# rain-neuromorphics/torchmx

Hardware: NVIDIA B200
Metric: to_mx/to_dtype GB/s (algorithmic bytes: quantize + dequantize->bf16, 16384x16384 bf16, all elem dtypes, block 32) (higher is better)
Workload: dtype u8 codes / f32 scaling arithmetic

## Files before the change

include/mxq.h:

```cpp
#ifndef MXQ_H_
#define MXQ_H_

#include <stdint.h>

#if defined(__GNUC__)
#define MXQ_API __attribute__((visibility("default")))
#else
#define MXQ_API
#endif

#ifdef __cplusplus
extern "C" {
#endif

typedef enum {
    MXQ_ELEM_E4M3 = 0,
    MXQ_ELEM_E3M2 = 1,
    MXQ_ELEM_E2M3 = 2,
    MXQ_ELEM_E2M1 = 3,
    MXQ_ELEM_INT8 = 4,
    MXQ_ELEM_E5M2 = 5
} mxq_elem_t;

typedef enum {
// ... 123 lines not shown
typedef struct {
    const void *x; int64_t n0, n1, rows, cols, s0, s1, row_stride;
    int elem ; unsigned flags ;
    void *codes; uint8_t *scales;
} mxq_transposed_quantize_args_t;
MXQ_API int mxq_quantize_transposed(const mxq_transposed_quantize_args_t *args, int device, void *stream);

#define MXQ_OK 0
#define MXQ_ERR_INVALID 1
#define MXQ_ERR_UNSUPPORTED_SHAPE 2
#define MXQ_ERR_CUDA 3

MXQ_API const char *mxq_last_error(void);
MXQ_API int mxq_version(void);
MXQ_API int mxq_arch(void);

#ifdef __cplusplus
}
#endif
#endif
```

torchmx_b200/_C.py:

```python
from __future__ import annotations

import ctypes
import os
import threading

_HERE = os.path.dirname(os.path.abspath(__file__))
LIB_PATH = os.path.join(_HERE, "lib", "libmxq.so")

OK, ERR_INVALID, ERR_UNSUPPORTED_SHAPE, ERR_CUDA = 0, 1, 2, 3
HP_BF16, HP_F32 = 0, 1
FLAG_HW_EXACT = 1
FLAG_OPERAND_LAYOUT = 2
GEMM_B_STATIC, GEMM_WIDE_TILES, GEMM_NO_PDL, GEMM_NO_MXF4 = 1, 2, 4, 8
ABI_VERSION = 3
MAX_DIMS = 6

EXPORTS = ("mxq_quantize", "mxq_dequantize", "mxq_dequantize_strided", "mxq_gemm", "mxq_gemm_dequant", "mxq_gemm_bf16", "mxq_transcode_to_e4m3", "mxq_pack_operand", "mxq_unpack_operand",
           "mxq_softmax_quantize", "mxq_flash_attention", "mxq_silu_mul_quantize", "mxq_rmsnorm", "mxq_rope", "mxq_quantize_heads", "mxq_quantize_transposed", "mxq_last_error", "mxq_version", "mxq_arch")


class GemmArgs(ctypes.Structure):
    _fields_ = [
        ("a_codes", ctypes.c_void_p), ("sfa", ctypes.c_void_p), ("lda", ctypes.c_int64), ("ld_sfa", ctypes.c_int64),
        ("a_batch_stride", ctypes.c_int64), ("sfa_batch_stride", ctypes.c_int64),
        ("b_codes", ctypes.c_void_p), ("sfb", ctypes.c_void_p), ("ldb", ctypes.c_int64), ("ld_sfb", ctypes.c_int64),
        ("b_batch_stride", ctypes.c_int64), ("sfb_batch_stride", ctypes.c_int64),
        ("bias", ctypes.c_void_p),
        ("d", ctypes.c_void_p), ("ldd", ctypes.c_int64), ("d_batch_stride", ctypes.c_int64),
        ("batch", ctypes.c_int64), ("M", ctypes.c_int64), ("N", ctypes.c_int64), ("K", ctypes.c_int64),
        ("a_format", ctypes.c_int), ("b_format", ctypes.c_int),
        ("d_multicast", ctypes.c_void_p),
        ("x_bf16", ctypes.c_void_p), ("ldx", ctypes.c_int64), ("x_quant_flags", ctypes.c_int),
        ("flags", ctypes.c_uint), ("split_k", ctypes.c_int),
# ... 90 lines not shown
    if _lib is not None:
        return _lib
    with _lock:
        if _lib is not None:
            return _lib
        if not os.path.exists(LIB_PATH):
            raise RuntimeError(
                f"torchmx_b200: {LIB_PATH} is missing. Build it with `python -m torchmx_b200.build` "
                "(needs nvcc; sm_100a). There is no CPU / PyTorch fallback for the MX kernels.")
        L = ctypes.CDLL(LIB_PATH)
        i64, i32, vp, u32 = ctypes.c_int64, ctypes.c_int, ctypes.c_void_p, ctypes.c_uint
        L.mxq_last_error.restype = ctypes.c_char_p
        L.mxq_last_error.argtypes = []
        L.mxq_version.restype = i32
        L.mxq_arch.restype = i32
        L.mxq_quantize.restype = i32
        L.mxq_quantize.argtypes = [vp, i32, i64, i32, i32, u32, vp, vp, i32, vp]
        L.mxq_dequantize.restype = i32
        L.mxq_dequantize.argtypes = [vp, vp, i64, i32, i32, i32, vp, i32, vp]
        L.mxq_dequantize_strided.restype = i32
        L.mxq_dequantize_strided.argtypes = [vp, vp, i32, ctypes.POINTER(i64), ctypes.POINTER(i64), ctypes.POINTER(i64),
                                             i32, i32, i32, i32, vp, i32, vp]
        L.mxq_gemm.restype = i32
        L.mxq_gemm.argtypes = [ctypes.POINTER(GemmArgs), i32, vp]
        L.mxq_gemm_dequant.restype = i32
        L.mxq_gemm_dequant.argtypes = [ctypes.POINTER(GemmDequantArgs), i32, vp]
        L.mxq_gemm_bf16.restype = i32
        L.mxq_gemm_bf16.argtypes = [vp, i64, i64, vp, i64, i64, vp, vp, i64, i64, i64, i64, i64, i64, i32, vp]
        L.mxq_transcode_to_e4m3.restype = i32
        L.mxq_transcode_to_e4m3.argtypes = [vp, i32, i64, vp, i32, vp]
# ... 34 lines not shown
```

torchmx_b200/csrc/mxq_api.cu:

```cuda
#include <cstdarg>
#include <cstdio>
#include <cstdlib>
#include <cstring>

#include "mxq_common.cuh"

namespace mxq {
cudaError_t launch_quantize(const void*, int, int64_t, int, int, unsigned, void*, uint8_t*, int, int, int, cudaStream_t);
cudaError_t launch_dequantize(const void*, const uint8_t*, int64_t, int, int, int, void*, int, int, int, cudaStream_t);
cudaError_t launch_dequantize_strided(const void*, const uint8_t*, int, const int64_t*, const int64_t*, const int64_t*, int, int, int, int,
                                      void*, cudaStream_t);
cudaError_t launch_transcode(const void*, int, int64_t, void*, int, cudaStream_t);
cudaError_t launch_pack_operand(const void*, int, int64_t, void*, int, cudaStream_t);
cudaError_t launch_unpack_operand(const void*, int, int64_t, void*, int, cudaStream_t);
int launch_gemm(const mxq_gemm_args_t*, int, int, cudaStream_t, char*, size_t);
namespace gemm { int launch_gemm_dequant(const mxq_gemm_dequant_args_t*, int, cudaStream_t, char*, size_t); }
namespace gemm { int launch_gemm_bf16(const void*, int64_t, int64_t, const void*, int64_t, int64_t, const void*, void*, int64_t, int64_t, int64_t, int64_t, int64_t, int64_t, int,
                                       cudaStream_t, char*, size_t); }
namespace gemm { int launch_flash_attention(const mxq_attention_args_t*, int, cudaStream_t, char*, size_t); }
cudaError_t launch_silu_mul_quantize(const void*, const void*, int64_t, int64_t, int64_t, int64_t, int, unsigned, void*, uint8_t*, int, cudaStream_t);
int launch_softmax_quantize(const mxq_softmax_args_t*, cudaStream_t, char*, size_t);
int launch_rmsnorm(const mxq_rmsnorm_args_t*, cudaStream_t, char*, size_t);
int launch_rope(const mxq_rope_args_t*, int, cudaStream_t, char*, size_t);
int launch_heads_quantize(const void*, int64_t, int64_t, int64_t, int64_t, int, unsigned, void*, uint8_t*, cudaStream_t, char*, size_t);
// ... 29 lines not shown
        if (prev >= 0 && cur != prev) cudaSetDevice(prev);
    }
};

int sm_count_of(int device) {
    static int cache[64];
    if (device >= 0 && device < 64 && cache[device]) return cache[device];
    int n = 0;
    if (cudaDeviceGetAttribute(&n, cudaDevAttrMultiProcessorCount, device) != cudaSuccess || n <= 0) n = 148;
    if (device >= 0 && device < 64) cache[device] = n;
    return n;
}

bool valid_elem(int e) { return e >= MXQ_ELEM_E4M3 && e <= MXQ_ELEM_E5M2; }

int env_int(const char* name) {
    const char* s = getenv(name);
    return s ? atoi(s) : 0;
}
int quant_ept_override() { static int v = env_int("MXQ_QUANT_EPT"); return (v == 8 || v == 16 || v == 32) ? v : 0; }
int deq_cb_override() { static int v = env_int("MXQ_DEQ_CB"); return (v == 16 || v == 32) ? v : 0; }
int waves_override() { static int v = env_int("MXQ_WAVES"); return v > 0 ? v : 0; }

}

extern "C" {

const char* mxq_last_error(void) { return g_err; }
int mxq_version(void) { return 3; }
int mxq_arch(void) { return 1000; }

int mxq_quantize(const void* src, int src_dtype, int64_t n_blocks, int block_size, int elem, unsigned flags, void* codes, uint8_t* scales,
                 int device, void* stream) {
    if (!valid_elem(elem)) return fail(MXQ_ERR_INVALID, "mxq_quantize: unknown element type %d", elem);
    if (src_dtype != MXQ_HP_BF16 && src_dtype != MXQ_HP_F32) return fail(MXQ_ERR_INVALID, "mxq_quantize: unsupported source dtype %d", src_dtype);
    if (n_blocks < 0 || block_size < 1) return fail(MXQ_ERR_INVALID, "mxq_quantize: bad n_blocks=%lld block_size=%d", (long long)n_blocks, block_size);
    if (n_blocks == 0) return MXQ_OK;
    if (!src || !codes || !scales) return fail(MXQ_ERR_INVALID, "mxq_quantize: null pointer");
    if (elem == MXQ_ELEM_E2M1 && ((n_blocks * block_size) & 1))
        return fail(MXQ_ERR_INVALID, "mxq_quantize: float4_e2m1 needs an even element count (got %lld)", (long long)(n_blocks * block_size));
    DeviceScope scope(device);
    if (scope.err != cudaSuccess) return fail_cuda(scope.err, "mxq_quantize: selecting device");
    const cudaError_t e = mxq::launch_quantize(src, src_dtype, n_blocks, block_size, elem, flags, codes, scales, sm_count_of(scope.cur),
                                               quant_ept_override(), waves_override(), (cudaStream_t)stream);
    if (e == cudaErrorNotSupported && (flags & MXQ_FLAG_OPERAND_LAYOUT))
        return fail(MXQ_ERR_UNSUPPORTED_SHAPE, "mxq_quantize: MXQ_FLAG_OPERAND_LAYOUT needs a 4 / 6-bit element type, block 32, bf16 source and 32-byte aligned pointers");
    return e == cudaSuccess ? MXQ_OK : fail_cuda(e, "mxq_quantize: launch");
}

int mxq_dequantize(const void* codes, const uint8_t* scales, int64_t n_blocks, int block_size, int elem, int dst_dtype, void* dst, int device,
                   void* stream) {
    if (!valid_elem(elem)) return fail(MXQ_ERR_INVALID, "mxq_dequantize: unknown element type %d", elem);
    if (dst_dtype != MXQ_HP_BF16 && dst_dtype != MXQ_HP_F32) return fail(MXQ_ERR_INVALID, "mxq_dequantize: unsupported target dtype %d", dst_dtype);
    if (n_blocks < 0 || block_size < 1) return fail(MXQ_ERR_INVALID, "mxq_dequantize: bad n_blocks=%lld block_size=%d", (long long)n_blocks, block_size);
    if (n_blocks == 0) return MXQ_OK;
    if (!codes || !scales || !dst) return fail(MXQ_ERR_INVALID, "mxq_dequantize: null pointer");
    if (elem == MXQ_ELEM_E2M1 && ((n_blocks * block_size) & 1)) return fail(MXQ_ERR_INVALID, "mxq_dequantize: float4_e2m1 needs an even element count");
    DeviceScope scope(device);
    if (scope.err != cudaSuccess) return fail_cuda(scope.err, "mxq_dequantize: selecting device");
    const cudaError_t e = mxq::launch_dequantize(codes, scales, n_blocks, block_size, elem, dst_dtype, dst, sm_count_of(scope.cur), deq_cb_override(), waves_override(),
                                                 (cudaStream_t)stream);
    return e == cudaSuccess ? MXQ_OK : fail_cuda(e, "mxq_dequantize: launch");
}

int mxq_dequantize_strided(const void* codes, const uint8_t* scales, int ndim, const int64_t* sizes, const int64_t* code_strides,
                           const int64_t* scale_strides, int block_dim, int block_size, int elem, int dst_dtype, void* dst, int device,
                           void* stream) {
    if (!valid_elem(elem)) return fail(MXQ_ERR_INVALID, "mxq_dequantize_strided: unknown element type %d", elem);
    if (dst_dtype != MXQ_HP_BF16 && dst_dtype != MXQ_HP_F32) return fail(MXQ_ERR_INVALID, "mxq_dequantize_strided: unsupported target dtype %d", dst_dtype);
    if (ndim < 1 || ndim > MXQ_MAX_DIMS) return fail(MXQ_ERR_INVALID, "mxq_dequantize_strided: ndim %d outside 1..%d", ndim, MXQ_MAX_DIMS);
    if (block_dim < 0 || block_dim >= ndim || block_size < 1) return fail(MXQ_ERR_INVALID, "mxq_dequantize_strided: bad block_dim=%d block_size=%d", block_dim, block_size);
    if (!sizes || !code_strides || !scale_strides) return fail(MXQ_ERR_INVALID, "mxq_dequantize_strided: null shape pointer");
    int64_t total = 1;
    for (int d = 0; d < ndim; ++d) {
        if (sizes[d] < 0) return fail(MXQ_ERR_INVALID, "mxq_dequantize_strided: negative size");
        total *= sizes[d];
// ... 189 lines not shown
```

torchmx_b200/csrc/mxq_common.cuh:

```cuda
#pragma once
#include <cstdlib>
#include <cstdint>
#include <cuda_runtime.h>

#include "../../include/mxq.h"

namespace mxq {

template <int ELEM> struct Fmt;
template <> struct Fmt<MXQ_ELEM_E4M3> { static constexpr int ebits = 4, mbits = 3, bias = 7, max_pow2 = 8; };
template <> struct Fmt<MXQ_ELEM_E3M2> { static constexpr int ebits = 3, mbits = 2, bias = 3, max_pow2 = 4; };
template <> struct Fmt<MXQ_ELEM_E2M3> { static constexpr int ebits = 2, mbits = 3, bias = 1, max_pow2 = 2; };
template <> struct Fmt<MXQ_ELEM_E2M1> { static constexpr int ebits = 2, mbits = 1, bias = 1, max_pow2 = 2; };
template <> struct Fmt<MXQ_ELEM_INT8> { static constexpr int ebits = 0, mbits = 7, bias = 0, max_pow2 = 6; };
template <> struct Fmt<MXQ_ELEM_E5M2> { static constexpr int ebits = 5, mbits = 2, bias = 15, max_pow2 = 15; };

struct alignas(32) u32x8 { uint32_t v[8]; };

__device__ __forceinline__ u32x8 ldg256_stream(const void* p) {
    u32x8 r;
    asm volatile("ld.global.nc.L1::no_allocate.v8.b32 {%0,%1,%2,%3,%4,%5,%6,%7}, [%8];"
                 : "=r"(r.v[0]), "=r"(r.v[1]), "=r"(r.v[2]), "=r"(r.v[3]), "=r"(r.v[4]), "=r"(r.v[5]), "=r"(r.v[6]), "=r"(r.v[7])
                 : "l"(p));
    return r;
// ... 7 lines not shown
    uint2 r;
    asm volatile("ld.global.nc.L1::no_allocate.v2.b32 {%0,%1}, [%2];" : "=r"(r.x), "=r"(r.y) : "l"(p));
    return r;
}
__device__ __forceinline__ void stg256_stream(void* p, const u32x8& r) {
    asm volatile("st.global.L1::no_allocate.v8.b32 [%0], {%1,%2,%3,%4,%5,%6,%7,%8};" ::"l"(p), "r"(r.v[0]), "r"(r.v[1]), "r"(r.v[2]),
                 "r"(r.v[3]), "r"(r.v[4]), "r"(r.v[5]), "r"(r.v[6]), "r"(r.v[7])
                 : "memory");
}
__device__ __forceinline__ void stg128_stream(void* p, uint4 r) {
    asm volatile("st.global.L1::no_allocate.v4.b32 [%0], {%1,%2,%3,%4};" ::"l"(p), "r"(r.x), "r"(r.y), "r"(r.z), "r"(r.w) : "memory");
}
__device__ __forceinline__ void stg64_stream(void* p, uint2 r) {
    asm volatile("st.global.L1::no_allocate.v2.b32 [%0], {%1,%2};" ::"l"(p), "r"(r.x), "r"(r.y) : "memory");
}

template <int ELEM>
__device__ __forceinline__ int shared_exp_from_maxE(int maxE) {
    int s = maxE - Fmt<ELEM>::max_pow2;
    s = max(s, 0);
    s = min(s, 254);
    return maxE == 255 ? 255 : s;
}
__device__ __forceinline__ float inv_scale_f32(int s) {
    return __uint_as_float(s <= 253 ? (uint32_t)(254 - s) << 23 : 0x00400000u);
}
__device__ __forceinline__ float scale_f32(int s) {
    return __uint_as_float(s == 0 ? 0x00400000u : (s == 255 ? 0x7FC00000u : (uint32_t)s << 23));
}

// ... 105 lines not shown
```

torchmx_b200/csrc/mxq_dequantize.cu:

```cuda
#include <type_traits>

#include "mxq_common.cuh"

namespace mxq {

constexpr int kDequantThreads = 256;

template <int ELEM>
__device__ __forceinline__ void decode4(uint32_t word, float sc, float (&f)[4]) {
    if constexpr (ELEM == MXQ_ELEM_INT8) {
#pragma unroll
        for (int j = 0; j < 4; ++j) f[j] = (float)(int)(int8_t)(word >> (8 * j)) * sc;
    } else {
        const uint32_t h0 = decode_pair_f16x2<ELEM>(word & 0xFFFF), h1 = decode_pair_f16x2<ELEM>(word >> 16);
        f[0] = f16lo_to_f32(h0) * sc; f[1] = f16hi_to_f32(h0) * sc;
        f[2] = f16lo_to_f32(h1) * sc; f[3] = f16hi_to_f32(h1) * sc;
    }
}

__device__ __forceinline__ void decode8_e2m1(uint32_t word, float sc, float (&f)[8]) {
#pragma unroll
    for (int j = 0; j < 4; ++j) {
        const uint32_t h = decode_e2m1_byte_f16x2((word >> (8 * j)) & 0xFF);
        f[2 * j] = f16hi_to_f32(h) * sc;
        f[2 * j + 1] = f16lo_to_f32(h) * sc;
    }
}

template <int N, bool F32>
__device__ __forceinline__ void store_run(void* dst, int64_t first_elem, const float (&f)[N]) {
    if constexpr (F32) {
        uint8_t* p = reinterpret_cast<uint8_t*>(dst) + first_elem * 4;
#pragma unroll
        for (int j = 0; j < N / 8; ++j) {
            u32x8 o;
#pragma unroll
            for (int k = 0; k < 8; ++k) o.v[k] = __float_as_uint(f[8 * j + k]);
            stg256_stream(p + 32 * j, o);
        }
    } else {
        uint8_t* p = reinterpret_cast<uint8_t*>(dst) + first_elem * 2;
#pragma unroll
        for (int j = 0; j < N / 16; ++j) {
            u32x8 o;
#pragma unroll
            for (int k = 0; k < 8; ++k) o.v[k] = pack_bf16x2(f[16 * j + 2 * k], f[16 * j + 2 * k + 1]);
            stg256_stream(p + 32 * j, o);
        }
    }
}

template <int ELEM, bool F32, int CB>
__global__ void __launch_bounds__(kDequantThreads) dequantize_b32_kernel(const uint8_t* __restrict__ codes, const uint8_t* __restrict__ scales,
                                                                         void* __restrict__ dst, int64_t n_code_bytes) {
    constexpr int PER = (ELEM == MXQ_ELEM_E2M1) ? 2 : 1;
    constexpr int NH = CB / 16;
    const int64_t n_chunks = n_code_bytes / CB;
    const int64_t stride = (int64_t)gridDim.x * kDequantThreads;
    for (int64_t c = (int64_t)blockIdx.x * kDequantThreads + threadIdx.x; c < n_chunks; c += stride) {
        uint32_t w[CB / 4];
        if constexpr (CB == 32) {
            const u32x8 v = ldg256_stream(codes + c * 32);
#pragma unroll
            for (int k = 0; k < 8; ++k) w[k] = v.v[k];
        } else {
            const uint4 v = ldg128_stream(codes + c * 16);
            w[0] = v.x; w[1] = v.y; w[2] = v.z; w[3] = v.w;
        }
        int s[NH];
#pragma unroll
        for (int h = 0; h < NH; ++h) s[h] = __ldg(scales + ((c * CB + 16 * h) * PER) / 32);
#pragma unroll
        for (int h = 0; h < NH; ++h) {
            const float sc = scale_f32(s[h]);
            const int64_t e0 = (c * CB + 16 * h) * PER;
            if constexpr (ELEM == MXQ_ELEM_E2M1) {
                float f[32];
#pragma unroll
                for (int i = 0; i < 4; ++i) {
                    float t[8];
                    decode8_e2m1(w[4 * h + i], sc, t);
#pragma unroll
                    for (int k = 0; k < 8; ++k) f[8 * i + k] = t[k];
                }
                store_run<32, F32>(dst, e0, f);
            } else {
                float f[16];
#pragma unroll
                for (int i = 0; i < 4; ++i) {
                    float t[4];
                    decode4<ELEM>(w[4 * h + i], sc, t);
#pragma unroll
                    for (int k = 0; k < 4; ++k) f[4 * i + k] = t[k];
                }
                store_run<16, F32>(dst, e0, f);
            }
        }
    }
}

struct StridedArgs {
    int ndim, block_dim, block_size;
    int64_t sizes[MXQ_MAX_DIMS], code_strides[MXQ_MAX_DIMS], scale_strides[MXQ_MAX_DIMS];
    int64_t total;
};

template <int ELEM, bool F32>
__global__ void dequantize_strided_kernel(const uint8_t* __restrict__ codes, const uint8_t* __restrict__ scales, void* __restrict__ dst,
                                          StridedArgs a) {
    const int64_t o = (int64_t)blockIdx.x * blockDim.x + threadIdx.x;
// ... 123 lines not shown
            const int chunk = ((q * PER) / CH + j) ^ (F32 ? 2 * g : g);
            const uint4 v = *reinterpret_cast<const uint4*>(&tile[kk][chunk * CH]);
            if (vec_out) {
                stg128_stream(out + j * CH, v);
            } else {
                const T* e = reinterpret_cast<const T*>(&v);
                for (int u = 0; u < CH; ++u)
                    if (n + j * CH + u < N) out[j * CH + u] = e[u];
            }
        }
    }
}

template <int ELEM, bool F32>
static cudaError_t launch_flat(const void* codes, const uint8_t* scales, int64_t n_blocks, int block_size, void* dst, int sm_count, int cb,
                               int waves, cudaStream_t stream) {
    if (n_blocks == 0) return cudaSuccess;
    if (block_size == 32 && ((uintptr_t)codes % 32) == 0 && ((uintptr_t)dst % 32) == 0) {
        const int64_t n_code_bytes = n_blocks * ((ELEM == MXQ_ELEM_E2M1) ? 16 : 32);
        if (cb != 16 && cb != 32) cb = (!F32 && ELEM != MXQ_ELEM_E2M1) ? 32 : 16;
        if (n_code_bytes % cb) cb = 16;
        const int64_t n_chunks = n_code_bytes / cb;
        const int64_t want = (n_chunks + kDequantThreads - 1) / kDequantThreads;
        const int64_t cap = waves > 0 ? (int64_t)sm_count * 8 * waves : (int64_t)0x7FFFFFFF;
        const int grid = (int)(want < cap ? want : cap);
        if (cb == 32) dequantize_b32_kernel<ELEM, F32, 32><<<grid, kDequantThreads, 0, stream>>>((const uint8_t*)codes, scales, dst, n_code_bytes);
        else dequantize_b32_kernel<ELEM, F32, 16><<<grid, kDequantThreads, 0, stream>>>((const uint8_t*)codes, scales, dst, n_code_bytes);
        return cudaGetLastError();
    }
    StridedArgs a{};
    a.ndim = 1; a.block_dim = 0; a.block_size = block_size;
    a.sizes[0] = n_blocks * block_size; a.code_strides[0] = 1; a.scale_strides[0] = 1;
    a.total = a.sizes[0];
    const unsigned grid = (unsigned)((a.total + 255) / 256);
    dequantize_strided_kernel<ELEM, F32><<<grid, 256, 0, stream>>>((const uint8_t*)codes, scales, dst, a);
    return cudaGetLastError();
}

template <int ELEM, bool F32>
static cudaError_t launch_strided(const void* codes, const uint8_t* scales, int ndim, const int64_t* sizes, const int64_t* cs,
                                  const int64_t* ss, int block_dim, int block_size, void* dst, cudaStream_t stream) {
    StridedArgs a{};
// ... 33 lines not shown
    return cudaGetLastError();
}

#define MXQ_DISPATCH_ELEM_DT(elem, f32, CALL)                                                    \
    switch (elem) {                                                                              \
    case MXQ_ELEM_E4M3: return f32 ? CALL(MXQ_ELEM_E4M3, true) : CALL(MXQ_ELEM_E4M3, false);     \
    case MXQ_ELEM_E3M2: return f32 ? CALL(MXQ_ELEM_E3M2, true) : CALL(MXQ_ELEM_E3M2, false);     \
    case MXQ_ELEM_E2M3: return f32 ? CALL(MXQ_ELEM_E2M3, true) : CALL(MXQ_ELEM_E2M3, false);     \
    case MXQ_ELEM_E2M1: return f32 ? CALL(MXQ_ELEM_E2M1, true) : CALL(MXQ_ELEM_E2M1, false);     \
    case MXQ_ELEM_INT8: return f32 ? CALL(MXQ_ELEM_INT8, true) : CALL(MXQ_ELEM_INT8, false);     \
    case MXQ_ELEM_E5M2: return f32 ? CALL(MXQ_ELEM_E5M2, true) : CALL(MXQ_ELEM_E5M2, false);     \
    default: return cudaErrorInvalidValue;                                                       \
    }

cudaError_t launch_dequantize(const void* codes, const uint8_t* scales, int64_t n_blocks, int block_size, int elem, int dst_dtype, void* dst,
                              int sm_count, int cb, int waves, cudaStream_t stream) {
    const bool f32 = dst_dtype == MXQ_HP_F32;
#define CALL(E, F) launch_flat<E, F>(codes, scales, n_blocks, block_size, dst, sm_count, cb, waves, stream)
    MXQ_DISPATCH_ELEM_DT(elem, f32, CALL)
#undef CALL
}

cudaError_t launch_dequantize_strided(const void* codes, const uint8_t* scales, int ndim, const int64_t* sizes, const int64_t* cs,
                                      const int64_t* ss, int block_dim, int block_size, int elem, int dst_dtype, void* dst,
                                      cudaStream_t stream) {
    const bool f32 = dst_dtype == MXQ_HP_F32;
#define CALL(E, F) launch_strided<E, F>(codes, scales, ndim, sizes, cs, ss, block_dim, block_size, dst, stream)
    MXQ_DISPATCH_ELEM_DT(elem, f32, CALL)
#undef CALL
}

}
```

torchmx_b200/csrc/mxq_quantize.cu:

```cuda
#include "mxq_quant_core.cuh"

namespace mxq {

constexpr int kQuantThreads = 256;

template <int ELEM, int EPT, int BS = 32, bool OPERAND = false>
__global__ void __launch_bounds__(kQuantThreads) quantize_b32_bf16_kernel(const uint16_t* __restrict__ src, uint8_t* __restrict__ codes,
                                                                           uint8_t* __restrict__ scales, int64_t n_blocks, uint32_t flags) {
    pdl_launch_dependents();
    constexpr int LPB = BS / EPT;
    constexpr int NW = EPT / 2;
    constexpr int NO = (ELEM == MXQ_ELEM_E2M1) ? NW / 4 : NW / 2;
    const int64_t n_chunks = n_blocks * LPB;
    const int64_t stride = (int64_t)gridDim.x * kQuantThreads;
    for (int64_t c0 = (int64_t)blockIdx.x * kQuantThreads; c0 < n_chunks; c0 += stride) {
        const int64_t c = c0 + threadIdx.x;
        const bool live = c < n_chunks;
        uint32_t w[NW];
        if (live) {
            const uint8_t* p = reinterpret_cast<const uint8_t*>(src) + c * (EPT * 2);
            if constexpr (EPT == 8) {
                const uint4 v = ldg128_stream(p);
                w[0] = v.x; w[1] = v.y; w[2] = v.z; w[3] = v.w;
            } else {
#pragma unroll
                for (int j = 0; j < NW / 8; ++j) {
                    const u32x8 v = ldg256_stream(p + 32 * j);
#pragma unroll
                    for (int k = 0; k < 8; ++k) w[8 * j + k] = v.v[k];
                }
            }
        } else {
#pragma unroll
            for (int i = 0; i < NW; ++i) w[i] = 0;
        }
        uint32_t m = 0;
#pragma unroll
        for (int i = 0; i < NW; ++i) m = umax16x2(m, w[i] & 0x7FFF7FFFu);
        m = max(m & 0xFFFFu, m >> 16);
#pragma unroll
        for (int d = 1; d < LPB; d <<= 1) m = max(m, __shfl_xor_sync(0xFFFFFFFFu, m, d));
        const int s = shared_exp_from_maxE<ELEM>((int)(m >> 7));
// ... 143 lines not shown
    const int64_t i = (int64_t)blockIdx.x * blockDim.x + threadIdx.x;
    if constexpr (ELEM == MXQ_ELEM_E2M1) {
        if (2 * i + 1 >= n_elems + 1) return;
        const int64_t e0 = 2 * i, e1 = 2 * i + 1;
        const uint32_t hi = code_generic<ELEM, T>(src[e0], scales[e0 / block_size], hw_exact);
        const uint32_t lo = code_generic<ELEM, T>(src[e1], scales[e1 / block_size], hw_exact);
        codes[i] = (uint8_t)((hi << 4) | lo);
    } else {
        if (i >= n_elems) return;
        codes[i] = (uint8_t)code_generic<ELEM, T>(src[i], scales[i / block_size], hw_exact);
    }
}

template <int ELEM>
static cudaError_t launch_quantize_elem(const void* src, int src_dtype, int64_t n_blocks, int block_size, unsigned flags, void* codes,
                                        uint8_t* scales, int sm_count, int ept_override, int waves, cudaStream_t stream) {
    if (n_blocks == 0) return cudaSuccess;
    const uintptr_t a_src = (uintptr_t)src, a_codes = (uintptr_t)codes;
    if (flags & MXQ_FLAG_OPERAND_LAYOUT) {
        if constexpr (ELEM == MXQ_ELEM_E2M1 || ELEM == MXQ_ELEM_E3M2 || ELEM == MXQ_ELEM_E2M3) {
            if (block_size != 32 || src_dtype != MXQ_HP_BF16 || (a_src % 32) || (a_codes % 32)) return cudaErrorNotSupported;
            const int64_t want = (n_blocks + kQuantThreads - 1) / kQuantThreads;
            const int grid = (int)(want < 0x7FFFFFFF ? want : 0x7FFFFFFF);
            quantize_b32_bf16_kernel<ELEM, 32, 32, true><<<grid, kQuantThreads, 0, stream>>>((const uint16_t*)src, (uint8_t*)codes, scales, n_blocks, flags);
            return cudaGetLastError();
        } else {
            return cudaErrorNotSupported;
        }
    }
    if (block_size == 32 && src_dtype == MXQ_HP_BF16 && (a_src % 32) == 0 && (a_codes % 32) == 0) {
        int ept = ept_override ? ept_override : 32;
        const int lpb = 32 / ept;
        const int64_t n_chunks = n_blocks * lpb;
        const int64_t want = (n_chunks + kQuantThreads - 1) / kQuantThreads;
        const int64_t cap = waves > 0 ? (int64_t)sm_count * 8 * waves : (int64_t)0x7FFFFFFF;
        const int grid = (int)(want < cap ? want : cap);
        const uint16_t* s16 = (const uint16_t*)src;
        uint8_t* c8 = (uint8_t*)codes;
        if (ept == 8) quantize_b32_bf16_kernel<ELEM, 8><<<grid, kQuantThreads, 0, stream>>>(s16, c8, scales, n_blocks, flags);
        else if (ept == 32) quantize_b32_bf16_kernel<ELEM, 32><<<grid, kQuantThreads, 0, stream>>>(s16, c8, scales, n_blocks, flags);
        else quantize_b32_bf16_kernel<ELEM, 16><<<grid, kQuantThreads, 0, stream>>>(s16, c8, scales, n_blocks, flags);
        return cudaGetLastError();
    }
    if (src_dtype == MXQ_HP_BF16 && (a_src % 32) == 0 && (a_codes % 32) == 0 && (block_size == 8 || block_size == 16 || block_size == 64 || block_size == 128)) {
        const int lpb = block_size <= 32 ? 1 : block_size / 32;
        const int64_t n_chunks = n_blocks * lpb;
        const int64_t want = (n_chunks + kQuantThreads - 1) / kQuantThreads;
        const int grid = (int)(want < 0x7FFFFFFF ? want : 0x7FFFFFFF);
        const uint16_t* s16 = (const uint16_t*)src;
        uint8_t* c8 = (uint8_t*)codes;
        if (block_size == 8) quantize_b32_bf16_kernel<ELEM, 8, 8><<<grid, kQuantThreads, 0, stream>>>(s16, c8, scales, n_blocks, flags);
        else if (block_size == 16) quantize_b32_bf16_kernel<ELEM, 16, 16><<<grid, kQuantThreads, 0, stream>>>(s16, c8, scales, n_blocks, flags);
        else if (block_size == 64) quantize_b32_bf16_kernel<ELEM, 32, 64><<<grid, kQuantThreads, 0, stream>>>(s16, c8, scales, n_blocks, flags);
        else quantize_b32_bf16_kernel<ELEM, 32, 128><<<grid, kQuantThreads, 0, stream>>>(s16, c8, scales, n_blocks, flags);
        return cudaGetLastError();
    }
    if (block_size == 32 && src_dtype == MXQ_HP_F32 && (a_src % 32) == 0 && (a_codes % 16) == 0) {
        const int64_t want = (n_blocks * 2 + kQuantThreads - 1) / kQuantThreads;
        const int grid = (int)(want < 0x7FFFFFFF ? want : 0x7FFFFFFF);
        quantize_b32_f32_kernel<ELEM><<<grid, kQuantThreads, 0, stream>>>((const float*)src, (uint8_t*)codes, scales, n_blocks);
        return cudaGetLastError();
    }
    const int64_t n_elems = n_blocks * block_size;
    const int threads = 256;
    const int64_t n_out = (ELEM == MXQ_ELEM_E2M1) ? n_elems / 2 : n_elems;
    const unsigned g1 = (unsigned)((n_blocks + threads - 1) / threads), g2 = (unsigned)((n_out + threads - 1) / threads);
    if (src_dtype == MXQ_HP_BF16) {
        scales_generic_kernel<ELEM, uint16_t><<<g1, threads, 0, stream>>>((const uint16_t*)src, scales, n_blocks, block_size);
        codes_generic_kernel<ELEM, uint16_t><<<g2, threads, 0, stream>>>((const uint16_t*)src, scales, (uint8_t*)codes, n_elems, block_size, flags);
    } else {
        scales_generic_kernel<ELEM, float><<<g1, threads, 0, stream>>>((const float*)src, scales, n_blocks, block_size);
        codes_generic_kernel<ELEM, float><<<g2, threads, 0, stream>>>((const float*)src, scales, (uint8_t*)codes, n_elems, block_size, flags);
    }
    return cudaGetLastError();
}

cudaError_t launch_quantize(const void* src, int src_dtype, int64_t n_blocks, int block_size, int elem, unsigned flags, void* codes,
                            uint8_t* scales, int sm_count, int ept_override, int waves, cudaStream_t stream) {
    switch (elem) {
    case MXQ_ELEM_E4M3: return launch_quantize_elem<MXQ_ELEM_E4M3>(src, src_dtype, n_blocks, block_size, flags, codes, scales, sm_count, ept_override, waves, stream);
    case MXQ_ELEM_E3M2: return launch_quantize_elem<MXQ_ELEM_E3M2>(src, src_dtype, n_blocks, block_size, flags, codes, scales, sm_count, ept_override, waves, stream);
    case MXQ_ELEM_E2M3: return launch_quantize_elem<MXQ_ELEM_E2M3>(src, src_dtype, n_blocks, block_size, flags, codes, scales, sm_count, ept_override, waves, stream);
    case MXQ_ELEM_E2M1: return launch_quantize_elem<MXQ_ELEM_E2M1>(src, src_dtype, n_blocks, block_size, flags, codes, scales, sm_count, ept_override, waves, stream);
    case MXQ_ELEM_INT8: return launch_quantize_elem<MXQ_ELEM_INT8>(src, src_dtype, n_blocks, block_size, flags, codes, scales, sm_count, ept_override, waves, stream);
    case MXQ_ELEM_E5M2: return launch_quantize_elem<MXQ_ELEM_E5M2>(src, src_dtype, n_blocks, block_size, flags, codes, scales, sm_count, ept_override, waves, stream);
    default: return cudaErrorInvalidValue;
    }
}

}
```

Baseline: 6533.

## Alternate quantize/dequantize traversal direction and add L2 evict-first hints for reuse

The host now records, per device, which source and code buffers the last large quantize touched and in which direction. The next kernel over the same buffers walks its tiles in reverse, so it starts on data still resident in L2 from the previous kernel. Streaming loads and stores also get an L2 evict_first cache policy, so the one-touch traffic does not push that reusable tail out of L2. In exchange it adds host-side global state behind a mutex, a new exported query function and an ABI version bump, and it depends on callers reusing pointers.

```diff
diff --git a/include/mxq.h b/include/mxq.h
--- a/include/mxq.h
+++ b/include/mxq.h
@@ -161,6 +161,7 @@
 MXQ_API const char *mxq_last_error(void);
 MXQ_API int mxq_version(void);
 MXQ_API int mxq_arch(void);
+MXQ_API int mxq_traversal_last(int device);
 
 #ifdef __cplusplus
 }
diff --git a/torchmx_b200/_C.py b/torchmx_b200/_C.py
--- a/torchmx_b200/_C.py
+++ b/torchmx_b200/_C.py
@@ -12,11 +12,11 @@
 FLAG_HW_EXACT = 1
 FLAG_OPERAND_LAYOUT = 2
 GEMM_B_STATIC, GEMM_WIDE_TILES, GEMM_NO_PDL, GEMM_NO_MXF4 = 1, 2, 4, 8
-ABI_VERSION = 3
+ABI_VERSION = 4
 MAX_DIMS = 6
 
 EXPORTS = ("mxq_quantize", "mxq_dequantize", "mxq_dequantize_strided", "mxq_gemm", "mxq_gemm_dequant", "mxq_gemm_bf16", "mxq_transcode_to_e4m3", "mxq_pack_operand", "mxq_unpack_operand",
-           "mxq_softmax_quantize", "mxq_flash_attention", "mxq_silu_mul_quantize", "mxq_rmsnorm", "mxq_rope", "mxq_quantize_heads", "mxq_quantize_transposed", "mxq_last_error", "mxq_version", "mxq_arch")
+           "mxq_softmax_quantize", "mxq_flash_attention", "mxq_silu_mul_quantize", "mxq_rmsnorm", "mxq_rope", "mxq_quantize_heads", "mxq_quantize_transposed", "mxq_last_error", "mxq_version", "mxq_arch", "mxq_traversal_last")
 
 
 class GemmArgs(ctypes.Structure):
@@ -137,6 +137,8 @@
         L.mxq_last_error.argtypes = []
         L.mxq_version.restype = i32
         L.mxq_arch.restype = i32
+        L.mxq_traversal_last.restype = i32
+        L.mxq_traversal_last.argtypes = [i32]
         L.mxq_quantize.restype = i32
         L.mxq_quantize.argtypes = [vp, i32, i64, i32, i32, u32, vp, vp, i32, vp]
         L.mxq_dequantize.restype = i32
diff --git a/torchmx_b200/csrc/mxq_api.cu b/torchmx_b200/csrc/mxq_api.cu
--- a/torchmx_b200/csrc/mxq_api.cu
+++ b/torchmx_b200/csrc/mxq_api.cu
@@ -2,12 +2,13 @@
 #include <cstdio>
 #include <cstdlib>
 #include <cstring>
+#include <mutex>
 
 #include "mxq_common.cuh"
 
 namespace mxq {
-cudaError_t launch_quantize(const void*, int, int64_t, int, int, unsigned, void*, uint8_t*, int, int, int, cudaStream_t);
-cudaError_t launch_dequantize(const void*, const uint8_t*, int64_t, int, int, int, void*, int, int, int, cudaStream_t);
+cudaError_t launch_quantize(const void*, int, int64_t, int, int, unsigned, void*, uint8_t*, int, int, int, int*, unsigned, cudaStream_t);
+cudaError_t launch_dequantize(const void*, const uint8_t*, int64_t, int, int, int, void*, int, int, int, int*, unsigned, cudaStream_t);
 cudaError_t launch_dequantize_strided(const void*, const uint8_t*, int, const int64_t*, const int64_t*, const int64_t*, int, int, int, int,
                                       void*, cudaStream_t);
 cudaError_t launch_transcode(const void*, int, int64_t, void*, int, cudaStream_t);
@@ -67,20 +68,59 @@
 
 bool valid_elem(int e) { return e >= MXQ_ELEM_E4M3 && e <= MXQ_ELEM_E5M2; }
 
-int env_int(const char* name) {
+int env_int(const char* name, int dflt = 0) {
     const char* s = getenv(name);
-    return s ? atoi(s) : 0;
+    return s ? atoi(s) : dflt;
 }
 int quant_ept_override() { static int v = env_int("MXQ_QUANT_EPT"); return (v == 8 || v == 16 || v == 32) ? v : 0; }
 int deq_cb_override() { static int v = env_int("MXQ_DEQ_CB"); return (v == 16 || v == 32) ? v : 0; }
 int waves_override() { static int v = env_int("MXQ_WAVES"); return v > 0 ? v : 0; }
+bool l2_order_enabled() { static bool v = env_int("MXQ_L2_ORDER", 1) != 0; return v; }
+unsigned l2_hints() { static unsigned v = (unsigned)env_int("MXQ_L2_HINTS", mxq::kHintK2Codes | mxq::kHintK2Out | mxq::kHintK1Src); return v; }
+
+constexpr int64_t kL2OrderMinBytes = 64ll << 20;
+constexpr int kMaxDevices = 64;
+struct K1Record {
+    const void* src = nullptr;
+    int64_t src_bytes = 0;
+    const void* codes = nullptr;
+    bool reversed = false;
+};
+std::mutex g_order_mu;
+K1Record g_k1[kMaxDevices];
+int g_last_order[kMaxDevices];
+
+bool quantize_order(int dev, const void* src, int64_t src_bytes, int64_t bytes) {
+    if (!l2_order_enabled() || bytes <= kL2OrderMinBytes || dev < 0 || dev >= kMaxDevices) return false;
+    std::lock_guard<std::mutex> lk(g_order_mu);
+    const K1Record& r = g_k1[dev];
+    return r.src == src && r.src_bytes == src_bytes && !r.reversed;
+}
+bool dequantize_order(int dev, const void* codes, int64_t bytes) {
+    if (!l2_order_enabled() || bytes <= kL2OrderMinBytes || dev < 0 || dev >= kMaxDevices) return false;
+    std::lock_guard<std::mutex> lk(g_order_mu);
+    return g_k1[dev].codes == codes && !g_k1[dev].reversed;
+}
+void record_order(int dev, int ran, bool k1, const void* src, int64_t src_bytes, const void* codes, int64_t bytes) {
+    if (ran < 0 || dev < 0 || dev >= kMaxDevices) return;
+    std::lock_guard<std::mutex> lk(g_order_mu);
+    const int bit = k1 ? 1 : 2;
+    g_last_order[dev] = ran ? (g_last_order[dev] | bit) : (g_last_order[dev] & ~bit);
+    if (k1 && bytes > kL2OrderMinBytes) g_k1[dev] = K1Record{src, src_bytes, codes, ran == 1};
+}
 
 }
 
 extern "C" {
 
 const char* mxq_last_error(void) { return g_err; }
-int mxq_version(void) { return 3; }
+int mxq_version(void) { return 4; }
+
+int mxq_traversal_last(int device) {
+    if (device < 0 || device >= kMaxDevices) return -1;
+    std::lock_guard<std::mutex> lk(g_order_mu);
+    return g_last_order[device];
+}
 int mxq_arch(void) { return 1000; }
 
 int mxq_quantize(const void* src, int src_dtype, int64_t n_blocks, int block_size, int elem, unsigned flags, void* codes, uint8_t* scales,
@@ -94,8 +134,13 @@
         return fail(MXQ_ERR_INVALID, "mxq_quantize: float4_e2m1 needs an even element count (got %lld)", (long long)(n_blocks * block_size));
     DeviceScope scope(device);
     if (scope.err != cudaSuccess) return fail_cuda(scope.err, "mxq_quantize: selecting device");
+    const int64_t n_elems = n_blocks * block_size;
+    const int64_t src_bytes = n_elems * (src_dtype == MXQ_HP_F32 ? 4 : 2);
+    const int64_t bytes = src_bytes + (elem == MXQ_ELEM_E2M1 ? n_elems / 2 : n_elems) + n_blocks;
+    int order = quantize_order(scope.cur, src, src_bytes, bytes);
     const cudaError_t e = mxq::launch_quantize(src, src_dtype, n_blocks, block_size, elem, flags, codes, scales, sm_count_of(scope.cur),
-                                               quant_ept_override(), waves_override(), (cudaStream_t)stream);
+                                               quant_ept_override(), waves_override(), &order, l2_hints(), (cudaStream_t)stream);
+    if (e == cudaSuccess) record_order(scope.cur, order, true, src, src_bytes, codes, bytes);
     if (e == cudaErrorNotSupported && (flags & MXQ_FLAG_OPERAND_LAYOUT))
         return fail(MXQ_ERR_UNSUPPORTED_SHAPE, "mxq_quantize: MXQ_FLAG_OPERAND_LAYOUT needs a 4 / 6-bit element type, block 32, bf16 source and 32-byte aligned pointers");
     return e == cudaSuccess ? MXQ_OK : fail_cuda(e, "mxq_quantize: launch");
@@ -111,8 +156,12 @@
     if (elem == MXQ_ELEM_E2M1 && ((n_blocks * block_size) & 1)) return fail(MXQ_ERR_INVALID, "mxq_dequantize: float4_e2m1 needs an even element count");
     DeviceScope scope(device);
     if (scope.err != cudaSuccess) return fail_cuda(scope.err, "mxq_dequantize: selecting device");
+    const int64_t n_elems = n_blocks * block_size;
+    const int64_t bytes = (elem == MXQ_ELEM_E2M1 ? n_elems / 2 : n_elems) + n_blocks + n_elems * (dst_dtype == MXQ_HP_F32 ? 4 : 2);
+    int order = dequantize_order(scope.cur, codes, bytes);
     const cudaError_t e = mxq::launch_dequantize(codes, scales, n_blocks, block_size, elem, dst_dtype, dst, sm_count_of(scope.cur), deq_cb_override(), waves_override(),
-                                                 (cudaStream_t)stream);
+                                                 &order, l2_hints(), (cudaStream_t)stream);
+    if (e == cudaSuccess) record_order(scope.cur, order, false, nullptr, 0, nullptr, bytes);
     return e == cudaSuccess ? MXQ_OK : fail_cuda(e, "mxq_dequantize: launch");
 }
 
diff --git a/torchmx_b200/csrc/mxq_common.cuh b/torchmx_b200/csrc/mxq_common.cuh
--- a/torchmx_b200/csrc/mxq_common.cuh
+++ b/torchmx_b200/csrc/mxq_common.cuh
@@ -45,6 +45,36 @@
 __device__ __forceinline__ void stg64_stream(void* p, uint2 r) {
     asm volatile("st.global.L1::no_allocate.v2.b32 [%0], {%1,%2};" ::"l"(p), "r"(r.x), "r"(r.y) : "memory");
 }
+
+__device__ __forceinline__ uint64_t l2_evict_first() {
+    uint64_t pol;
+    asm volatile("createpolicy.fractional.L2::evict_first.b64 %0, 1.0;" : "=l"(pol));
+    return pol;
+}
+__device__ __forceinline__ u32x8 ldg256_stream(const void* p, uint64_t pol) {
+    u32x8 r;
+    asm volatile("ld.global.nc.L1::no_allocate.L2::cache_hint.v8.b32 {%0,%1,%2,%3,%4,%5,%6,%7}, [%8], %9;"
+                 : "=r"(r.v[0]), "=r"(r.v[1]), "=r"(r.v[2]), "=r"(r.v[3]), "=r"(r.v[4]), "=r"(r.v[5]), "=r"(r.v[6]), "=r"(r.v[7])
+                 : "l"(p), "l"(pol));
+    return r;
+}
+__device__ __forceinline__ uint4 ldg128_stream(const void* p, uint64_t pol) {
+    uint4 r;
+    asm volatile("ld.global.nc.L1::no_allocate.L2::cache_hint.v4.b32 {%0,%1,%2,%3}, [%4], %5;" : "=r"(r.x), "=r"(r.y), "=r"(r.z), "=r"(r.w)
+                 : "l"(p), "l"(pol));
+    return r;
+}
+__device__ __forceinline__ void stg256_stream(void* p, const u32x8& r, uint64_t pol) {
+    asm volatile("st.global.L1::no_allocate.L2::cache_hint.v8.b32 [%0], {%1,%2,%3,%4,%5,%6,%7,%8}, %9;" ::"l"(p), "r"(r.v[0]), "r"(r.v[1]),
+                 "r"(r.v[2]), "r"(r.v[3]), "r"(r.v[4]), "r"(r.v[5]), "r"(r.v[6]), "r"(r.v[7]), "l"(pol)
+                 : "memory");
+}
+
+enum : unsigned {
+    kHintK2Codes = 1,
+    kHintK2Out = 2,
+    kHintK1Src = 4,
+};
 
 template <int ELEM>
 __device__ __forceinline__ int shared_exp_from_maxE(int maxE) {
diff --git a/torchmx_b200/csrc/mxq_dequantize.cu b/torchmx_b200/csrc/mxq_dequantize.cu
--- a/torchmx_b200/csrc/mxq_dequantize.cu
+++ b/torchmx_b200/csrc/mxq_dequantize.cu
@@ -28,7 +28,7 @@
 }
 
 template <int N, bool F32>
-__device__ __forceinline__ void store_run(void* dst, int64_t first_elem, const float (&f)[N]) {
+__device__ __forceinline__ void store_run(void* dst, int64_t first_elem, const float (&f)[N], bool hint, uint64_t pol) {
     if constexpr (F32) {
         uint8_t* p = reinterpret_cast<uint8_t*>(dst) + first_elem * 4;
 #pragma unroll
@@ -36,7 +36,8 @@
             u32x8 o;
 #pragma unroll
             for (int k = 0; k < 8; ++k) o.v[k] = __float_as_uint(f[8 * j + k]);
-            stg256_stream(p + 32 * j, o);
+            if (hint) stg256_stream(p + 32 * j, o, pol);
+            else stg256_stream(p + 32 * j, o);
         }
     } else {
         uint8_t* p = reinterpret_cast<uint8_t*>(dst) + first_elem * 2;
@@ -45,26 +46,31 @@
             u32x8 o;
 #pragma unroll
             for (int k = 0; k < 8; ++k) o.v[k] = pack_bf16x2(f[16 * j + 2 * k], f[16 * j + 2 * k + 1]);
-            stg256_stream(p + 32 * j, o);
+            if (hint) stg256_stream(p + 32 * j, o, pol);
+            else stg256_stream(p + 32 * j, o);
         }
     }
 }
 
 template <int ELEM, bool F32, int CB>
 __global__ void __launch_bounds__(kDequantThreads) dequantize_b32_kernel(const uint8_t* __restrict__ codes, const uint8_t* __restrict__ scales,
-                                                                         void* __restrict__ dst, int64_t n_code_bytes) {
+                                                                         void* __restrict__ dst, int64_t n_code_bytes, bool reverse, unsigned hints) {
     constexpr int PER = (ELEM == MXQ_ELEM_E2M1) ? 2 : 1;
     constexpr int NH = CB / 16;
     const int64_t n_chunks = n_code_bytes / CB;
-    const int64_t stride = (int64_t)gridDim.x * kDequantThreads;
-    for (int64_t c = (int64_t)blockIdx.x * kDequantThreads + threadIdx.x; c < n_chunks; c += stride) {
+    const int64_t n_tiles = (n_chunks + kDequantThreads - 1) / kDequantThreads;
+    const bool hint_codes = (hints & kHintK2Codes) != 0, hint_out = (hints & kHintK2Out) != 0;
+    const uint64_t pol = hints ? l2_evict_first() : 0;
+    for (int64_t tile = blockIdx.x; tile < n_tiles; tile += gridDim.x) {
+        const int64_t c = (reverse ? n_tiles - 1 - tile : tile) * kDequantThreads + threadIdx.x;
+        if (c >= n_chunks) continue;
         uint32_t w[CB / 4];
         if constexpr (CB == 32) {
-            const u32x8 v = ldg256_stream(codes + c * 32);
+            const u32x8 v = hint_codes ? ldg256_stream(codes + c * 32, pol) : ldg256_stream(codes + c * 32);
 #pragma unroll
             for (int k = 0; k < 8; ++k) w[k] = v.v[k];
         } else {
-            const uint4 v = ldg128_stream(codes + c * 16);
+            const uint4 v = hint_codes ? ldg128_stream(codes + c * 16, pol) : ldg128_stream(codes + c * 16);
             w[0] = v.x; w[1] = v.y; w[2] = v.z; w[3] = v.w;
         }
         int s[NH];
@@ -83,7 +89,7 @@
 #pragma unroll
                     for (int k = 0; k < 8; ++k) f[8 * i + k] = t[k];
                 }
-                store_run<32, F32>(dst, e0, f);
+                store_run<32, F32>(dst, e0, f, hint_out, pol);
             } else {
                 float f[16];
 #pragma unroll
@@ -93,7 +99,7 @@
 #pragma unroll
                     for (int k = 0; k < 4; ++k) f[4 * i + k] = t[k];
                 }
-                store_run<16, F32>(dst, e0, f);
+                store_run<16, F32>(dst, e0, f, hint_out, pol);
             }
         }
     }
@@ -247,7 +253,9 @@
 
 template <int ELEM, bool F32>
 static cudaError_t launch_flat(const void* codes, const uint8_t* scales, int64_t n_blocks, int block_size, void* dst, int sm_count, int cb,
-                               int waves, cudaStream_t stream) {
+                               int waves, int* order, unsigned hints, cudaStream_t stream) {
+    const bool rev = *order == 1;
+    *order = -1;
     if (n_blocks == 0) return cudaSuccess;
     if (block_size == 32 && ((uintptr_t)codes % 32) == 0 && ((uintptr_t)dst % 32) == 0) {
         const int64_t n_code_bytes = n_blocks * ((ELEM == MXQ_ELEM_E2M1) ? 16 : 32);
@@ -257,8 +265,10 @@
         const int64_t want = (n_chunks + kDequantThreads - 1) / kDequantThreads;
         const int64_t cap = waves > 0 ? (int64_t)sm_count * 8 * waves : (int64_t)0x7FFFFFFF;
         const int grid = (int)(want < cap ? want : cap);
-        if (cb == 32) dequantize_b32_kernel<ELEM, F32, 32><<<grid, kDequantThreads, 0, stream>>>((const uint8_t*)codes, scales, dst, n_code_bytes);
-        else dequantize_b32_kernel<ELEM, F32, 16><<<grid, kDequantThreads, 0, stream>>>((const uint8_t*)codes, scales, dst, n_code_bytes);
+        hints &= kHintK2Codes | kHintK2Out;
+        if (cb == 32) dequantize_b32_kernel<ELEM, F32, 32><<<grid, kDequantThreads, 0, stream>>>((const uint8_t*)codes, scales, dst, n_code_bytes, rev, hints);
+        else dequantize_b32_kernel<ELEM, F32, 16><<<grid, kDequantThreads, 0, stream>>>((const uint8_t*)codes, scales, dst, n_code_bytes, rev, hints);
+        *order = rev;
         return cudaGetLastError();
     }
     StridedArgs a{};
@@ -322,9 +332,9 @@
     }
 
 cudaError_t launch_dequantize(const void* codes, const uint8_t* scales, int64_t n_blocks, int block_size, int elem, int dst_dtype, void* dst,
-                              int sm_count, int cb, int waves, cudaStream_t stream) {
+                              int sm_count, int cb, int waves, int* order, unsigned hints, cudaStream_t stream) {
     const bool f32 = dst_dtype == MXQ_HP_F32;
-#define CALL(E, F) launch_flat<E, F>(codes, scales, n_blocks, block_size, dst, sm_count, cb, waves, stream)
+#define CALL(E, F) launch_flat<E, F>(codes, scales, n_blocks, block_size, dst, sm_count, cb, waves, order, hints, stream)
     MXQ_DISPATCH_ELEM_DT(elem, f32, CALL)
 #undef CALL
 }
diff --git a/torchmx_b200/csrc/mxq_quantize.cu b/torchmx_b200/csrc/mxq_quantize.cu
--- a/torchmx_b200/csrc/mxq_quantize.cu
+++ b/torchmx_b200/csrc/mxq_quantize.cu
@@ -6,26 +6,28 @@
 
 template <int ELEM, int EPT, int BS = 32, bool OPERAND = false>
 __global__ void __launch_bounds__(kQuantThreads) quantize_b32_bf16_kernel(const uint16_t* __restrict__ src, uint8_t* __restrict__ codes,
-                                                                           uint8_t* __restrict__ scales, int64_t n_blocks, uint32_t flags) {
+                                                                           uint8_t* __restrict__ scales, int64_t n_blocks, uint32_t flags,
+                                                                           bool reverse, bool hint_src) {
     pdl_launch_dependents();
     constexpr int LPB = BS / EPT;
     constexpr int NW = EPT / 2;
     constexpr int NO = (ELEM == MXQ_ELEM_E2M1) ? NW / 4 : NW / 2;
     const int64_t n_chunks = n_blocks * LPB;
-    const int64_t stride = (int64_t)gridDim.x * kQuantThreads;
-    for (int64_t c0 = (int64_t)blockIdx.x * kQuantThreads; c0 < n_chunks; c0 += stride) {
-        const int64_t c = c0 + threadIdx.x;
+    const int64_t n_tiles = (n_chunks + kQuantThreads - 1) / kQuantThreads;
+    const uint64_t pol = hint_src ? l2_evict_first() : 0;
+    for (int64_t tile = blockIdx.x; tile < n_tiles; tile += gridDim.x) {
+        const int64_t c = (reverse ? n_tiles - 1 - tile : tile) * kQuantThreads + threadIdx.x;
         const bool live = c < n_chunks;
         uint32_t w[NW];
         if (live) {
             const uint8_t* p = reinterpret_cast<const uint8_t*>(src) + c * (EPT * 2);
             if constexpr (EPT == 8) {
-                const uint4 v = ldg128_stream(p);
+                const uint4 v = hint_src ? ldg128_stream(p, pol) : ldg128_stream(p);
                 w[0] = v.x; w[1] = v.y; w[2] = v.z; w[3] = v.w;
             } else {
 #pragma unroll
                 for (int j = 0; j < NW / 8; ++j) {
-                    const u32x8 v = ldg256_stream(p + 32 * j);
+                    const u32x8 v = hint_src ? ldg256_stream(p + 32 * j, pol) : ldg256_stream(p + 32 * j);
 #pragma unroll
                     for (int k = 0; k < 8; ++k) w[8 * j + k] = v.v[k];
                 }
@@ -199,7 +201,10 @@
 
 template <int ELEM>
 static cudaError_t launch_quantize_elem(const void* src, int src_dtype, int64_t n_blocks, int block_size, unsigned flags, void* codes,
-                                        uint8_t* scales, int sm_count, int ept_override, int waves, cudaStream_t stream) {
+                                        uint8_t* scales, int sm_count, int ept_override, int waves, int* order, unsigned hints,
+                                        cudaStream_t stream) {
+    const bool rev = *order == 1, hint = (hints & kHintK1Src) != 0;
+    *order = -1;
     if (n_blocks == 0) return cudaSuccess;
     const uintptr_t a_src = (uintptr_t)src, a_codes = (uintptr_t)codes;
     if (flags & MXQ_FLAG_OPERAND_LAYOUT) {
@@ -207,7 +212,7 @@
             if (block_size != 32 || src_dtype != MXQ_HP_BF16 || (a_src % 32) || (a_codes % 32)) return cudaErrorNotSupported;
             const int64_t want = (n_blocks + kQuantThreads - 1) / kQuantThreads;
             const int grid = (int)(want < 0x7FFFFFFF ? want : 0x7FFFFFFF);
-            quantize_b32_bf16_kernel<ELEM, 32, 32, true><<<grid, kQuantThreads, 0, stream>>>((const uint16_t*)src, (uint8_t*)codes, scales, n_blocks, flags);
+            quantize_b32_bf16_kernel<ELEM, 32, 32, true><<<grid, kQuantThreads, 0, stream>>>((const uint16_t*)src, (uint8_t*)codes, scales, n_blocks, flags, false, false);
             return cudaGetLastError();
         } else {
             return cudaErrorNotSupported;
@@ -222,9 +227,10 @@
         const int grid = (int)(want < cap ? want : cap);
         const uint16_t* s16 = (const uint16_t*)src;
         uint8_t* c8 = (uint8_t*)codes;
-        if (ept == 8) quantize_b32_bf16_kernel<ELEM, 8><<<grid, kQuantThreads, 0, stream>>>(s16, c8, scales, n_blocks, flags);
-        else if (ept == 32) quantize_b32_bf16_kernel<ELEM, 32><<<grid, kQuantThreads, 0, stream>>>(s16, c8, scales, n_blocks, flags);
-        else quantize_b32_bf16_kernel<ELEM, 16><<<grid, kQuantThreads, 0, stream>>>(s16, c8, scales, n_blocks, flags);
+        if (ept == 8) quantize_b32_bf16_kernel<ELEM, 8><<<grid, kQuantThreads, 0, stream>>>(s16, c8, scales, n_blocks, flags, rev, hint);
+        else if (ept == 32) quantize_b32_bf16_kernel<ELEM, 32><<<grid, kQuantThreads, 0, stream>>>(s16, c8, scales, n_blocks, flags, rev, hint);
+        else quantize_b32_bf16_kernel<ELEM, 16><<<grid, kQuantThreads, 0, stream>>>(s16, c8, scales, n_blocks, flags, rev, hint);
+        *order = rev;
         return cudaGetLastError();
     }
     if (src_dtype == MXQ_HP_BF16 && (a_src % 32) == 0 && (a_codes % 32) == 0 && (block_size == 8 || block_size == 16 || block_size == 64 || block_size == 128)) {
@@ -234,10 +240,11 @@
         const int grid = (int)(want < 0x7FFFFFFF ? want : 0x7FFFFFFF);
         const uint16_t* s16 = (const uint16_t*)src;
         uint8_t* c8 = (uint8_t*)codes;
-        if (block_size == 8) quantize_b32_bf16_kernel<ELEM, 8, 8><<<grid, kQuantThreads, 0, stream>>>(s16, c8, scales, n_blocks, flags);
-        else if (block_size == 16) quantize_b32_bf16_kernel<ELEM, 16, 16><<<grid, kQuantThreads, 0, stream>>>(s16, c8, scales, n_blocks, flags);
-        else if (block_size == 64) quantize_b32_bf16_kernel<ELEM, 32, 64><<<grid, kQuantThreads, 0, stream>>>(s16, c8, scales, n_blocks, flags);
-        else quantize_b32_bf16_kernel<ELEM, 32, 128><<<grid, kQuantThreads, 0, stream>>>(s16, c8, scales, n_blocks, flags);
+        if (block_size == 8) quantize_b32_bf16_kernel<ELEM, 8, 8><<<grid, kQuantThreads, 0, stream>>>(s16, c8, scales, n_blocks, flags, rev, hint);
+        else if (block_size == 16) quantize_b32_bf16_kernel<ELEM, 16, 16><<<grid, kQuantThreads, 0, stream>>>(s16, c8, scales, n_blocks, flags, rev, hint);
+        else if (block_size == 64) quantize_b32_bf16_kernel<ELEM, 32, 64><<<grid, kQuantThreads, 0, stream>>>(s16, c8, scales, n_blocks, flags, rev, hint);
+        else quantize_b32_bf16_kernel<ELEM, 32, 128><<<grid, kQuantThreads, 0, stream>>>(s16, c8, scales, n_blocks, flags, rev, hint);
+        *order = rev;
         return cudaGetLastError();
     }
     if (block_size == 32 && src_dtype == MXQ_HP_F32 && (a_src % 32) == 0 && (a_codes % 16) == 0) {
@@ -261,14 +268,14 @@
 }
 
 cudaError_t launch_quantize(const void* src, int src_dtype, int64_t n_blocks, int block_size, int elem, unsigned flags, void* codes,
-                            uint8_t* scales, int sm_count, int ept_override, int waves, cudaStream_t stream) {
+                            uint8_t* scales, int sm_count, int ept_override, int waves, int* order, unsigned hints, cudaStream_t stream) {
     switch (elem) {
-    case MXQ_ELEM_E4M3: return launch_quantize_elem<MXQ_ELEM_E4M3>(src, src_dtype, n_blocks, block_size, flags, codes, scales, sm_count, ept_override, waves, stream);
-    case MXQ_ELEM_E3M2: return launch_quantize_elem<MXQ_ELEM_E3M2>(src, src_dtype, n_blocks, block_size, flags, codes, scales, sm_count, ept_override, waves, stream);
-    case MXQ_ELEM_E2M3: return launch_quantize_elem<MXQ_ELEM_E2M3>(src, src_dtype, n_blocks, block_size, flags, codes, scales, sm_count, ept_override, waves, stream);
-    case MXQ_ELEM_E2M1: return launch_quantize_elem<MXQ_ELEM_E2M1>(src, src_dtype, n_blocks, block_size, flags, codes, scales, sm_count, ept_override, waves, stream);
-    case MXQ_ELEM_INT8: return launch_quantize_elem<MXQ_ELEM_INT8>(src, src_dtype, n_blocks, block_size, flags, codes, scales, sm_count, ept_override, waves, stream);
-    case MXQ_ELEM_E5M2: return launch_quantize_elem<MXQ_ELEM_E5M2>(src, src_dtype, n_blocks, block_size, flags, codes, scales, sm_count, ept_override, waves, stream);
+    case MXQ_ELEM_E4M3: return launch_quantize_elem<MXQ_ELEM_E4M3>(src, src_dtype, n_blocks, block_size, flags, codes, scales, sm_count, ept_override, waves, order, hints, stream);
+    case MXQ_ELEM_E3M2: return launch_quantize_elem<MXQ_ELEM_E3M2>(src, src_dtype, n_blocks, block_size, flags, codes, scales, sm_count, ept_override, waves, order, hints, stream);
+    case MXQ_ELEM_E2M3: return launch_quantize_elem<MXQ_ELEM_E2M3>(src, src_dtype, n_blocks, block_size, flags, codes, scales, sm_count, ept_override, waves, order, hints, stream);
+    case MXQ_ELEM_E2M1: return launch_quantize_elem<MXQ_ELEM_E2M1>(src, src_dtype, n_blocks, block_size, flags, codes, scales, sm_count, ept_override, waves, order, hints, stream);
+    case MXQ_ELEM_INT8: return launch_quantize_elem<MXQ_ELEM_INT8>(src, src_dtype, n_blocks, block_size, flags, codes, scales, sm_count, ept_override, waves, order, hints, stream);
+    case MXQ_ELEM_E5M2: return launch_quantize_elem<MXQ_ELEM_E5M2>(src, src_dtype, n_blocks, block_size, flags, codes, scales, sm_count, ept_override, waves, order, hints, stream);
     default: return cudaErrorInvalidValue;
     }
 }
```

Result: faster. 6689 (median of 6 runs) (+2.4%).
